# rahulaggarwal965/vslam

Measured on AMD Instinct MI355X. Metric: frame-pairs/sec (extract+match+RANSAC) @1280×720, 2k kp, 4096 hyp; 1/2/4/8 GPU, higher is better.
Workload: dtype u8/f32/f64; 1 GPU; C3: 1280x720, 2000 keypoints, 4096 hypotheses, batch 256 pairs per GPU, SURVEY 8(d) data: rotation + parallax, sub-pixel resampling, 40-45 % outlier matches; pairs_per_gpu=256, batches_in_flight=4

## Files before the change

vslam_amd/build.py:

```python
import os
import subprocess
import sys

HERE = os.path.dirname(os.path.abspath(__file__))
CSRC = os.path.join(HERE, "csrc")
LIB = os.path.join(HERE, "libvslam_amd.so")
SOURCES = ["capi.hip", "match.hip", "ransac_sets.hip", "ransac_solve.hip", "ransac_count.hip", "ransac_prune.hip", "ransac_select.hip", "refit.hip", "refine.hip",
           "kdtree.hip", "gray.hip", "response.hip", "select.hip", "blur.hip",
           "brief.hip", "orb_grid.hip", "pose.hip", "assoc.hip", "map.hip", "world.hip", "resect.hip", "adjust.hip", "search.hip", "render.hip", "multi.hip", "pipeline.hip"]
HEADERS = ["ctx.h", "introselect.h", "image_common.h", "ransac_svd.h", "ransac_residual.h", "ransac_prune_cert.h", "block_reduce.h", "lm_math.h", "refine_math.h", "resect_math.h", "adjust_math.h", "search_math.h", "world_select.h", "world_match.h",
           os.path.join("..", "..", "include", "vslam_amd.h"),
           os.path.join("..", "..", "include", "vslam_resect.h"),
           os.path.join("..", "..", "include", "vslam_adjust.h"),
           os.path.join("..", "..", "include", "vslam_search.h"),
           os.path.join("..", "..", "include", "vslam_brief_pattern_31.h")]
FLAGS = ["--offload-arch=gfx950", "-O3", "-std=c++17", "-ffp-contract=off", "-fPIC", "-Wall"]
EXTRA_FLAGS = {"response.hip": ["-fno-slp-vectorize"]}
OBJDIR = os.path.join(HERE, "_obj")


EXP_LIB = os.path.join(HERE, "libvslam_amd_exp.so")
EXP_OBJDIR = os.path.join(HERE, "_obj_exp")


def _compile(hipcc, src, verbose, objdir=None, extra=()):
# ... 64 lines not shown
```

vslam_amd/capi.py:

```python
import ctypes as C
import os

_HERE = os.path.dirname(os.path.abspath(__file__))
LIB_PATH = os.environ.get("VSLAM_AMD_LIB") or os.path.join(_HERE, "libvslam_amd.so")
EXP_LIB_PATH = os.path.join(_HERE, "libvslam_amd_exp.so")

OK = 0
ERRORS = {-1: "VSLAM_ERR_INVALID", -2: "VSLAM_ERR_HIP", -3: "VSLAM_ERR_NO_DEVICE",
          -4: "VSLAM_ERR_CAPACITY", -5: "VSLAM_ERR_DEGENERATE", -6: "VSLAM_ERR_COMM"}

SYMBOLS = [
    "vslam_ctx_create", "vslam_ctx_make_current", "vslam_ctx_destroy", "vslam_ctx_set_stream", "vslam_ctx_set_option", "vslam_ctx_synchronize", "vslam_ctx_wait",
    "vslam_last_error", "vslam_ctx_workspace_bytes", "vslam_version", "vslam_brief_pattern_31", "vslam_dev_alloc", "vslam_dev_free", "vslam_copy_h2d",
    "vslam_copy_d2h", "vslam_debug_stream_copy", "vslam_debug_valu_calib", "vslam_prof_enable", "vslam_prof_reset", "vslam_prof_count", "vslam_prof_get",
    "vslam_match_knn2_ratio", "vslam_ransac_sets", "vslam_ransac_fundamental", "vslam_ransac_solve",
    "vslam_ransac_evaluate", "vslam_refit_fundamental", "vslam_refine_pairs", "vslam_kdtree_build",
    "vslam_kdtree_radius", "vslam_kdtree_nearest", "vslam_kdtree_cell_table", "vslam_extract_features", "vslam_extract_features_grid", "vslam_triangulate_points", "vslam_frontend_pairs_pose", "vslam_pipeline_batches_redone", "vslam_corner_stats", "vslam_bgr2gray", "vslam_min_eigen",
    "vslam_good_features", "vslam_gaussian7", "vslam_orb_describe", "vslam_extract_Rt", "vslam_triangulate", "vslam_associate_map_points", "vslam_reprojection_filter",
    "vslam_match_features",
    "vslam_map_create", "vslam_map_destroy", "vslam_map_reset", "vslam_map_step", "vslam_map_view", "vslam_map_observations",
    "vslam_track_sequences",
    "vslam_world_create", "vslam_world_destroy", "vslam_world_reset", "vslam_world_step", "vslam_world_lift", "vslam_world_view",
    "vslam_map_attach_world", "vslam_world_render",
    "vslam_view_default", "vslam_view_look_at", "vslam_render_points", "vslam_map_render",
# ... 255 lines not shown
        W = width if width is not None else bgr.shape[2]
        stride = bgr.shape[2] * (bgr.shape[3] if bgr.dim() == 4 else 1)
        xy = torch.zeros((F, max_corners, 2), dtype=torch.float32, device=bgr.device)
        n = torch.zeros((F,), dtype=torch.int32, device=bgr.device)
        self._ready()
        self._check(self.lib.vslam_debug_detect(self.handle, _ptr(bgr), C.c_int(F), C.c_int(W), C.c_int(H), C.c_int(stride),
                                                C.c_int(max_corners), C.c_int(max_corners), _ptr(xy), _ptr(n)))
        return xy, n

    def debug_ransac_prune_x(self, batch, hyp):
        torch = self.torch
        x = torch.zeros((batch, hyp), dtype=torch.int32, device="cuda")
        self._ready()
        self._check(self.lib.vslam_debug_ransac_prune_x(self.handle, _ptr(x), C.c_int(batch), C.c_int(hyp)))
        return x

    def debug_ransac_prune_tile(self, F, xy):
        torch = self.torch
        self._dev(F, torch.float32, "F"); self._dev(xy, torch.float32, "xy")
        assert tuple(F.shape) == (32, 9) and tuple(xy.shape) == (4, 32)
        n = torch.zeros((32, 32), dtype=torch.float32, device=F.device)
        a0 = torch.zeros((32, 32), dtype=torch.float32, device=F.device)
        self._ready()
        self._check(self.lib.vslam_debug_ransac_prune_tile(self.handle, _ptr(F), _ptr(xy), _ptr(n), _ptr(a0)))
        return n, a0

    def debug_valu_calib(self):
        self._check(self.lib.vslam_debug_valu_calib(self.handle))

    def debug_stream_copy(self, src, dst, bytes_per_lane):
# ... 1016 lines not shown
```

vslam_amd/csrc/match.hip:

```cpp
#include "ctx.h"

#include <cstdlib>

namespace {

constexpr int kThreads = 256;
#ifdef VSLAM_EXPERIMENTS
constexpr int kQueriesPerLane = 2;
constexpr int kTile = 256;

__device__ __forceinline__ uint32_t bcnt_acc(uint32_t x, uint32_t acc) {
    uint32_t r;
    asm("v_bcnt_u32_b32 %0, %1, %2" : "=v"(r) : "v"(x), "v"(acc));
    return r;
}
__device__ __forceinline__ uint32_t med3_u32(uint32_t a, uint32_t b, uint32_t c) {
    uint32_t r;
    asm("v_med3_u32 %0, %1, %2, %3" : "=v"(r) : "v"(a), "v"(b), "v"(c));
    return r;
}
__device__ __forceinline__ uint32_t ham256(const uint4 &qa, const uint4 &qb, const uint4 &ta,
                                           const uint4 &tb) {
    uint32_t d = bcnt_acc(qa.x ^ ta.x, 0u);
    d = bcnt_acc(qa.y ^ ta.y, d);
// ... 265 lines not shown
                int4 o;
                o.x = nt >= 1 ? i0 : -1;
                o.y = nt >= 1 ? d0 : 0x7FFFFFFF;
                o.z = nt >= 2 ? i1 : -1;
                o.w = nt >= 2 ? d1 : 0x7FFFFFFF;
                knn_b[q] = o;
            }
        }
}

#endif

typedef int v8i __attribute__((ext_vector_type(8)));
typedef float v16f __attribute__((ext_vector_type(16)));
constexpr int kFStride = 144;
constexpr float kFScale = 16384.f;
constexpr float kFPad = 33554432.f;
constexpr float kFNone = -67108864.f;
constexpr int kFBias = 0x05000000;

__device__ __forceinline__ uint32_t spread8_pm1(uint32_t b) {
    uint32_t x = (b | (b << 12)) & 0x000F000Fu;
    x = (x | (x << 6)) & 0x03030303u;
    x = (x | (x << 3)) & 0x11111111u;
    return (x << 3) | 0x22222222u;
}
__device__ __forceinline__ v4i spread32_pm1(uint32_t w) {
    v4i r;
    r.x = (int)spread8_pm1(w & 0xFFu);
    r.y = (int)spread8_pm1((w >> 8) & 0xFFu);
    r.z = (int)spread8_pm1((w >> 16) & 0xFFu);
    r.w = (int)spread8_pm1(w >> 24);
    return r;
}
__device__ __forceinline__ float med3_f32(float a, float b, float c) { return __builtin_amdgcn_fmed3f(a, b, c); }

__global__ __launch_bounds__(256) void match_spread_kernel(const uint8_t *__restrict__ desc2, const int32_t *__restrict__ n2,
                                                           int kp_stride, int kp_pad, uint8_t *__restrict__ tx) {
    const int b = blockIdx.y, i = blockIdx.x * 256 + threadIdx.x;
    const int row = i >> 3;
    if (row >= n2[b]) return;
    const uint32_t w = reinterpret_cast<const uint32_t *>(desc2 + (size_t)b * kp_stride * VSLAM_DESC_BYTES)[i];
    *reinterpret_cast<v4i *>(tx + ((size_t)b * kp_pad + row) * 128 + (size_t)(i & 7) * 16) = spread32_pm1(w);
}

template <int RT, bool PRE, int CT>
__global__ __launch_bounds__(64 * kMQ / (32 * RT)) void match_knn2_fp4_kernel(
    const uint8_t *__restrict__ desc1, const int32_t *__restrict__ n1, const uint8_t *__restrict__ desc2,
    const int32_t *__restrict__ n2, int kp_stride, int32_t *__restrict__ sel, int32_t *__restrict__ knn,
    const uint8_t *__restrict__ tx, int kp_pad, int batch, int per_pair) {
    int b, qt;
    vs_xcd_item_block(blockIdx.x, per_pair, b, qt);
    if (b >= batch) return;
    const int tid = threadIdx.x, lane = tid & 63;
    const int wave = __builtin_amdgcn_readfirstlane(tid >> 6);
    const int nq = n1[b], nt = n2[b];
    const int qbase = qt * kMQ;
    if (qbase >= nq) return;

    static_assert(CT == 1 || PRE, "two tiles per trip only with pre-spread train rows");
    __shared__ __align__(16) uint8_t s_b[2][CT * kMT * kFStride];
    const uint32_t *q32 = reinterpret_cast<const uint32_t *>(desc1 + (size_t)b * kp_stride * VSLAM_DESC_BYTES);
    const uint32_t *t32 = reinterpret_cast<const uint32_t *>(desc2 + (size_t)b * kp_stride * VSLAM_DESC_BYTES);
    int32_t *sel_b = sel + (size_t)b * kp_stride;
    int4 *knn_b = knn ? reinterpret_cast<int4 *>(knn) + (size_t)b * kp_stride : nullptr;

    const int r = lane & 31, half = lane >> 5;
    v8i a[RT][4];
#pragma unroll
    for (int rt = 0; rt < RT; rt++) {
        const int q = min(qbase + wave * (32 * RT) + rt * 32 + r, nq - 1);
        const uint2 *qrow = reinterpret_cast<const uint2 *>(q32 + (size_t)q * 8);
#pragma unroll
        for (int s = 0; s < 4; s++) {
            const uint2 w2 = qrow[s];
            const v4i x = spread32_pm1(half ? w2.y : w2.x);
// ... 2 lines not shown
    }
    float k1[RT][16], k2[RT][16];
#pragma unroll
    for (int rt = 0; rt < RT; rt++)
#pragma unroll
        for (int g = 0; g < 16; g++) {
            k1[rt][g] = kFNone;
            k2[rt][g] = kFNone;
        }

    constexpr bool kSplit = RT == 1;
    const int st = kSplit ? (tid & 255) : tid, shalf = kSplit ? (tid >> 8) : 0;
    const int srow = st >> 3, sd = st & 7;
    struct Stage {
        uint4 v[CT];
    };
    const uint8_t *txb = PRE ? tx + (size_t)b * kp_pad * 128 + (size_t)srow * 128 + sd * 16 + (kSplit ? 8 * shalf : 0) : nullptr;
    auto fetch = [&](int trip) -> Stage {
        Stage st_;
#pragma unroll
        for (int c = 0; c < CT; c++) {
            uint4 v = make_uint4(0u, 0u, 0u, 0u);
            if (PRE) {
                const uint8_t *src = txb + (size_t)(trip * CT + c) * (kMT * 128);
                if (kSplit) {
                    const uint2 h = *reinterpret_cast<const uint2 *>(src);
                    v.x = h.x;
                    v.y = h.y;
                } else {
                    v = *reinterpret_cast<const uint4 *>(src);
                }
            } else {
                const int t = trip * kMT + srow;
                v.x = t < nt ? t32[(size_t)t * 8 + sd] : 0u;
            }
            st_.v[c] = v;
        }
        return st_;
    };
    auto expand = [&](const Stage &st_, int buf) {
#pragma unroll
        for (int c = 0; c < CT; c++) {
            const uint4 v = st_.v[c];
            uint8_t *dst = &s_b[buf][(c * kMT + srow) * kFStride + sd * 16];
            if (PRE) {
                if (kSplit) *reinterpret_cast<uint2 *>(dst + 8 * shalf) = make_uint2(v.x, v.y);
                else *reinterpret_cast<uint4 *>(dst) = v;
            } else if (kSplit) {
                const uint32_t hw = (v.x >> (16 * shalf)) & 0xFFFFu;
                *reinterpret_cast<uint2 *>(dst + 8 * shalf) = make_uint2(spread8_pm1(hw & 0xFFu), spread8_pm1(hw >> 8));
            } else {
                *reinterpret_cast<v4i *>(dst) = spread32_pm1(v.x);
            }
        }
    };

    const int ntrips = (nt + CT * kMT - 1) / (CT * kMT);
    if (ntrips > 0) expand(fetch(0), 0);
    Stage w_next;
    if (ntrips > 1) w_next = fetch(1);
    __syncthreads();
    for (int trip = 0; trip < ntrips; trip++) {
        const int buf = trip & 1;
        if (trip + 1 < ntrips) expand(w_next, buf ^ 1);
        if (trip + 2 < ntrips) w_next = fetch(trip + 2);
        v16f acc[CT][RT];
#pragma unroll
        for (int c = 0; c < CT; c++) {
#pragma unroll
            for (int rt = 0; rt < RT; rt++) acc[c][rt] = v16f{0, 0, 0, 0, 0, 0, 0, 0, 0, 0, 0, 0, 0, 0, 0, 0};
            const uint8_t *src = &s_b[buf][(c * kMT + r) * kFStride + 16 * half];
#pragma unroll
            for (int s = 0; s < 4; s++) {
                const v4i bq = *reinterpret_cast<const v4i *>(src + 32 * s);
                const v8i bv = v8i{bq.x, bq.y, bq.z, bq.w, 0, 0, 0, 0};
#pragma unroll
                for (int rt = 0; rt < RT; rt++)
                    acc[c][rt] = __builtin_amdgcn_mfma_scale_f32_32x32x64_f8f6f4(a[rt][s], bv, acc[c][rt], 4, 4, 0, 0x7F7F7F7F, 0, 0x7F7F7F7F);
            }
        }
#pragma unroll
        for (int c = 0; c < CT; c++) {
            const int t = (trip * CT + c) * kMT + r;
            const float nidx = t < nt ? -(float)t : -kFPad;
#pragma unroll
            for (int g = 0; g < 16; g++) {
#pragma unroll
                for (int rt = 0; rt < RT; rt++) {
                    const float key = __builtin_fmaf(acc[c][rt][g], kFScale, nidx);
                    k2[rt][g] = med3_f32(k1[rt][g], k2[rt][g], key);
                    k1[rt][g] = fmaxf(k1[rt][g], key);
                }
            }
        }
        __syncthreads();
    }

#pragma unroll
    for (int rt = 0; rt < RT; rt++)
#pragma unroll
        for (int g = 0; g < 16; g++) {
            uint32_t x1 = (uint32_t)(kFBias - (int)k1[rt][g]), x2 = (uint32_t)(kFBias - (int)k2[rt][g]);
            merge2<0xB1>(x1, x2);
            merge2<0x4E>(x1, x2);
// ... 70 lines not shown
                    const int32_t *n2, int batch, int kp_stride, int32_t *pairs, int32_t *m,
                    int32_t *knn) {
    VS_REQUIRE(ctx, d1 && n1 && d2 && n2 && pairs && m, VSLAM_ERR_INVALID);
    VS_REQUIRE(ctx, batch > 0 && kp_stride > 0, VSLAM_ERR_INVALID);
    VS_REQUIRE(ctx, kp_stride <= VSLAM_MAX_KP, VSLAM_ERR_CAPACITY);
    int32_t *sel = nullptr;
    int rc = vs_arena_get(ctx, "match.sel", sizeof(int32_t) * (size_t)batch * kp_stride, (void **)&sel);
    if (rc) return rc;
#ifndef VSLAM_EXPERIMENTS
    {
        VsProfScope ps(ctx, "match_knn2_kernel");
        const int per_pair = vs_div_up(kp_stride, kMQ);
        const int xgrid = vs_xcd_grid(batch, per_pair);
        const int kp_pad = vs_div_up(kp_stride, 2 * kMT) * 2 * kMT;
        uint8_t *tx = nullptr;
        if ((rc = vs_arena_get(ctx, "match.spread", (size_t)batch * kp_pad * 128, (void **)&tx))) return rc;
        match_spread_kernel<<<dim3(vs_div_up(kp_stride * 8, 256), batch), 256, 0, ctx->stream>>>(d2, n2, kp_stride, kp_pad, tx);
        match_knn2_fp4_kernel<1, true, 2><<<xgrid, 512, 0, ctx->stream>>>(d1, n1, d2, n2, kp_stride, sel, knn, tx, kp_pad, batch, per_pair);
    }
#else
    static const bool popcount_path = VS_EXPERIMENT_ENV("VSLAM_MATCH_POPCOUNT") != nullptr;
    {
        VsProfScope ps(ctx, "match_knn2_kernel");
        if (popcount_path) {
            dim3 grid(vs_div_up(kp_stride, kThreads * kQueriesPerLane), batch);
            match_knn2_kernel<<<grid, kThreads, 0, ctx->stream>>>(d1, n1, d2, n2, kp_stride, sel, knn);
        } else {
            static const char *const shape = VS_EXPERIMENT_ENV("VSLAM_MATCH_SHAPE");
#ifdef VSLAM_EXPERIMENTS
            const int pick = ctx->match_shape ? ctx->match_shape : (shape ? (shape[0] == '4' ? 2 : 1) : 0);
#else
            constexpr int pick = 0;
            (void)shape;
// ... 2 lines not shown
            dim3 grid(vs_div_up(kp_stride, kMQ), batch);
            static const char *const form = VS_EXPERIMENT_ENV("VSLAM_MATCH_FORM");
#ifdef VSLAM_EXPERIMENTS
            const bool fp4 = ctx->match_form ? ctx->match_form == 1 : !(form && form[0] == 'i');
#else
            constexpr bool fp4 = true;
            (void)form;
#endif
            if (fp4) {
                const bool wide4 = pick == 2;
                const int per_pair = vs_div_up(kp_stride, kMQ);
                const int xgrid = vs_xcd_grid(batch, per_pair);
                static const char *const nopre = VS_EXPERIMENT_ENV("VSLAM_MATCH_NO_PRESPREAD");
                static const char *const ct_env = VS_EXPERIMENT_ENV("VSLAM_MATCH_TILES_PER_TRIP");
                const int ct = ct_env ? atoi(ct_env) : 2;
                if (!nopre) {
                    const int kp_pad = vs_div_up(kp_stride, 2 * kMT) * 2 * kMT;
                    uint8_t *tx = nullptr;
                    if ((rc = vs_arena_get(ctx, "match.spread", (size_t)batch * kp_pad * 128, (void **)&tx))) return rc;
                    match_spread_kernel<<<dim3(vs_div_up(kp_stride * 8, 256), batch), 256, 0, ctx->stream>>>(d2, n2, kp_stride, kp_pad, tx);
                    if (wide4 && ct == 2) match_knn2_fp4_kernel<2, true, 2><<<xgrid, 256, 0, ctx->stream>>>(d1, n1, d2, n2, kp_stride, sel, knn, tx, kp_pad, batch, per_pair);
                    else if (wide4) match_knn2_fp4_kernel<2, true, 1><<<xgrid, 256, 0, ctx->stream>>>(d1, n1, d2, n2, kp_stride, sel, knn, tx, kp_pad, batch, per_pair);
                    else if (ct == 2) match_knn2_fp4_kernel<1, true, 2><<<xgrid, 512, 0, ctx->stream>>>(d1, n1, d2, n2, kp_stride, sel, knn, tx, kp_pad, batch, per_pair);
                    else match_knn2_fp4_kernel<1, true, 1><<<xgrid, 512, 0, ctx->stream>>>(d1, n1, d2, n2, kp_stride, sel, knn, tx, kp_pad, batch, per_pair);
                } else if (wide4) {
                    match_knn2_fp4_kernel<2, false, 1><<<xgrid, 256, 0, ctx->stream>>>(d1, n1, d2, n2, kp_stride, sel, knn, nullptr, 0, batch, per_pair);
                } else {
                    match_knn2_fp4_kernel<1, false, 1><<<xgrid, 512, 0, ctx->stream>>>(d1, n1, d2, n2, kp_stride, sel, knn, nullptr, 0, batch, per_pair);
                }
            } else if (wide) match_knn2_mfma_kernel<2><<<grid, 256, 0, ctx->stream>>>(d1, n1, d2, n2, kp_stride, sel, knn);
            else match_knn2_mfma_kernel<1><<<grid, 512, 0, ctx->stream>>>(d1, n1, d2, n2, kp_stride, sel, knn);
        }
    }
#endif
    {
        VsProfScope ps(ctx, "match_compact_kernel");
        match_compact_kernel<<<batch, kThreads, 0, ctx->stream>>>(sel, n1, kp_stride, pairs, m);
    }
    VS_HIP(ctx, hipGetLastError());
    return VSLAM_OK;
}
```

vslam_amd/csrc/ransac_count.hip:

```cpp
#include "ransac_residual.h"

namespace {
using namespace vs_ransac;

constexpr int kCntHyps = 128;
constexpr int kCntWaves = 8;
constexpr int kCntQueue = 320;
constexpr int kCntLdsMatches = 4096;
constexpr int kScreenMatches = 128;
constexpr int kScreenHyps = 128;
constexpr int kRankThreads = 512;
constexpr int kPilotHyps = kRankThreads / 64;
constexpr int kCandMax = 8;
constexpr float kCntTinyDD = 0x1p-120f;
constexpr int kFcmpOGT = 2, kFcmpOLT = 4, kFcmpULT = 12;
constexpr int kCntRec = 12;
typedef __attribute__((address_space(3))) volatile uint32_t cnt_queue_t;
static_assert(VSLAM_MAX_KP <= 65536, "queue words keep the match index in 16 bits");

__host__ __device__ constexpr int cnt_pad(int n) { return (n + 255) & ~255; }
constexpr int kHeadUncertified = -1;
__device__ __forceinline__ float cnt_sum_rel(int adds) { return fmaxf(0x1p-18f, (float)(13 + adds) * 0x1p-24f); }

struct CntBand {
    float lo, hi;
    double beta;
    bool ok;
};
__device__ __forceinline__ CntBand cnt_band(const float *f, float C1, float C2, float threshold) {
    CntBand B;
    bool ok = threshold >= 0x1p-20f && threshold <= 0x1p20f && C1 <= 0x1p20f && C2 <= 0x1p20f;
#pragma unroll
    for (int k = 0; k < 9; k++) ok = ok && fabsf(f[k]) <= 1024.f;
    const double S = ((double)fabsf(f[0]) + (double)fabsf(f[3]) + (double)fabsf(f[1]) + (double)fabsf(f[4])) * (double)C2 +
                     (double)fabsf(f[6]) + (double)fabsf(f[7]);
    const double beta = 4.04 * 0x1p-24 * S + 1e-30;
// ... 317 lines not shown
            r[2 * kp_pad + pos] = c.x;
            r[3 * kp_pad + pos] = c.y;
        }
    }
    const int mpad = cnt_pad(m);
    if (m + tid < mpad) {
        const int2 pr = PR[m - 1];
        const float2 a = P1[pr.x], c = P2[pr.y];
        r[m + tid] = a.x;
        r[kp_pad + m + tid] = a.y;
        r[2 * kp_pad + m + tid] = c.x;
        r[3 * kp_pad + m + tid] = c.y;
    }
}

__global__ __launch_bounds__(256) void ransac_screen_kernel(
    const float *__restrict__ rk, int kp_pad, const int32_t *__restrict__ m_arr, int min_m, int kp_stride, int hyp,
    float threshold, const float *__restrict__ hypF, const float *__restrict__ cmax, const int32_t *__restrict__ cbound,
    int32_t *__restrict__ pot0, int2 *__restrict__ head) {
    const int b = blockIdx.y, tid = threadIdx.x, lane = tid & 63;
    const int wave = __builtin_amdgcn_readfirstlane(tid >> 6);
    const int hbase = blockIdx.x * kScreenHyps;
    const int m = min(m_arr[b], kp_stride);
    if (m < min_m) return;
    __shared__ __align__(16) float s_rec[kScreenHyps * kCntRec];
    if (tid < kScreenHyps) {
        const float *src = hypF + ((size_t)b * hyp + min(hbase + tid, hyp - 1)) * 9;
        float f[9];
#pragma unroll
        for (int k = 0; k < 9; k++) f[k] = src[k];
        const CntBand B = cnt_band(f, cmax[2 * b], cmax[2 * b + 1], threshold);
        cnt_store_record(s_rec + tid * kCntRec, f, B);
    }
    const int n0 = min(m, kScreenMatches);
    const int bound_pilots = cbound[b];
    const float *r = rk + (size_t)b * 4 * kp_pad;
    const float2 x1 = *reinterpret_cast<const float2 *>(r + 2 * lane);
    const float2 y1 = *reinterpret_cast<const float2 *>(r + kp_pad + 2 * lane);
    const float2 x2 = *reinterpret_cast<const float2 *>(r + 2 * kp_pad + 2 * lane);
    const float2 y2 = *reinterpret_cast<const float2 *>(r + 3 * kp_pad + 2 * lane);
    v2f X1, Y1, X2, Y2;
    X1.x = x1.x; X1.y = x1.y; Y1.x = y1.x; Y1.y = y1.y;
    X2.x = x2.x; X2.y = x2.y; Y2.x = y2.x; Y2.y = y2.y;
    const unsigned long long va = __ballot(2 * lane < n0), vb = __ballot(2 * lane + 1 < n0);
    __syncthreads();
    int mine = 0;
    float mine_sum = 0.f;
    const bool odd1 = (lane & 1) != 0, odd2 = (lane & 2) != 0;
    const bool in_a = 2 * lane < n0, in_b = 2 * lane + 1 < n0;
    constexpr int kU = 4;
// ... 411 lines not shown
    const bool from_zero = VS_EXPERIMENT_ENV("VSLAM_RANSAC_COUNT_FROM_ZERO") != nullptr;
#ifdef VSLAM_EXPERIMENTS
    const int exit_payload = VS_EXPERIMENT_ENV("VSLAM_RANSAC_COUNT_EXIT_PAYLOAD") != nullptr ? 1 : 0;
#endif
    int2 *head = nullptr;
    if ((rc = vs_arena_get(ctx, "ransac.head", sizeof(int2) * (size_t)batch * hyp, (void **)&head))) return rc;
    const unsigned long long *use_floor = no_sum_rule ? nullptr : sfloor;
    if ((rc = vs_arena_get(ctx, "ransac.pot0", sizeof(int32_t) * (size_t)batch * hyp, (void **)&pot0))) return rc;
    if ((rc = vs_arena_get(ctx, "ransac.rk", sizeof(float) * 4 * (size_t)kp_pad * batch, (void **)&rk))) return rc;
    if ((rc = vs_arena_get(ctx, "ransac.cmax", sizeof(float) * 2 * (size_t)batch, (void **)&cmax))) return rc;
    {
        VsProfScope ps(ctx, "ransac_rank_kernel");
        ransac_rank_kernel<<<batch, kRankThreads, 0, ctx->stream>>>(xy1, xy2, pairs, m, min_m, kp_stride, kp_pad, hyp, threshold, hypF,
                                                                    cbound, rk, cmax, sfloor);
    }
    {
        VsProfScope ps(ctx, "ransac_screen_kernel");
        dim3 grid(vs_div_up(hyp, kScreenHyps), batch);
        ransac_screen_kernel<<<grid, 256, 0, ctx->stream>>>(rk, kp_pad, m, min_m, kp_stride, hyp, threshold, hypF, cmax, cbound, pot0, head);
    }
    {
        VsProfScope ps(ctx, "ransac_cand_kernel");
        ransac_cand_kernel<<<batch, 64 * kCandMax, 0, ctx->stream>>>(rk, kp_pad, m, min_m, kp_stride, hyp, threshold, hypF, pot0,
                                                                     no_sum_rule ? 0 : 1, cbound, sfloor);
    }
    if ((rc = vs_launch_ransac_prune(ctx, rk, kp_pad, m, min_m, kp_stride, hyp, threshold, hypF, cmax, cbound, pot0, batch, kScreenMatches)))
        return rc;
    if (int arc = vs_aux_job_point(ctx, 4)) return arc;
    {
        VsProfScope ps(ctx, "ransac_count_kernel");
        const bool lds = kp_pad <= kCntLdsMatches;
        const size_t dyn = (lds ? sizeof(float) * 4 * (size_t)kp_pad : 0) + sizeof(uint32_t) * kCntQueue * kCntWaves;
        const size_t dyn_max = sizeof(float) * 4 * kCntLdsMatches + sizeof(uint32_t) * kCntQueue * kCntWaves;
        dim3 grid(vs_div_up(hyp, kCntHyps), batch);
#ifdef VSLAM_EXPERIMENTS
// ... 30 lines not shown
```

vslam_amd/csrc/ransac_prune.hip:

```cpp
#include "ransac_prune_cert.h"
#include "ransac_residual.h"

namespace {

typedef float v16f __attribute__((ext_vector_type(16)));
constexpr int kPruneWaves = 4;
constexpr int kPruneHyps = 32;
constexpr int kPruneTile = 32;
constexpr int kPruneStep = 2;
constexpr int kPruneOGT = 2;

__host__ __device__ constexpr int prune_row(int r, int half) { return (r & 3) + 8 * (r >> 2) + 4 * half; }

struct PruneA {
    float n[5], d[2];
};
__device__ __forceinline__ PruneA prune_operands(const float *f, bool half) {
    PruneA A;
#pragma unroll
    for (int s = 0; s < 4; s++) A.n[s] = half ? f[2 * s + 1] : f[2 * s];
    A.n[4] = half ? 0.f : f[8];
    A.d[0] = half ? f[1] : f[0];
    A.d[1] = half ? 0.f : f[2];
    return A;
}

__device__ __forceinline__ void prune_tile(const PruneA &A, bool half, float x1, float y1, float x2, float y2, v16f &n, v16f &a0) {
    const float p = x2 * (half ? y1 : x1);
    const float q = y2 * (half ? x1 : y1);
    const float b1 = half ? q : x2, b2 = half ? y2 : q, b3 = half ? y1 : x1, b4 = half ? 0.f : 1.f;
    v16f z;
#pragma unroll
    for (int r = 0; r < 16; r++) z[r] = 0.f;
    n = __builtin_amdgcn_mfma_f32_32x32x2f32(A.n[0], p, z, 0, 0, 0);
    n = __builtin_amdgcn_mfma_f32_32x32x2f32(A.n[1], b1, n, 0, 0, 0);
    n = __builtin_amdgcn_mfma_f32_32x32x2f32(A.n[2], b2, n, 0, 0, 0);
    n = __builtin_amdgcn_mfma_f32_32x32x2f32(A.n[3], b3, n, 0, 0, 0);
    n = __builtin_amdgcn_mfma_f32_32x32x2f32(A.n[4], b4, n, 0, 0, 0);
    a0 = __builtin_amdgcn_mfma_f32_32x32x2f32(A.d[0], b3, z, 0, 0, 0);
    a0 = __builtin_amdgcn_mfma_f32_32x32x2f32(A.d[1], b4, a0, 0, 0, 0);
}

#ifdef VSLAM_EXPERIMENTS
#define VS_PRUNE_X_PARAM , int32_t *__restrict__ x_out
#else
#define VS_PRUNE_X_PARAM
#endif

__global__ __launch_bounds__(64 * kPruneWaves) void ransac_prune_mfma_kernel(
    const float *__restrict__ rk, int kp_pad, const int32_t *__restrict__ m_arr, int min_m, int kp_stride, int hyp, float threshold,
    float splus, const float *__restrict__ hypF, const float *__restrict__ cmax, const int32_t *__restrict__ cbound, int32_t *__restrict__ pot0,
    int n_head, int gate VS_PRUNE_X_PARAM) {
    const int b = blockIdx.y, lane = threadIdx.x & 63, col = lane & 31;
    const bool half = lane >= 32;
    const int wave = __builtin_amdgcn_readfirstlane(threadIdx.x >> 6);
    const int m = min(m_arr[b], kp_stride);
// ... 113 lines not shown
#endif
    return VSLAM_OK;
}

#ifdef VSLAM_EXPERIMENTS
extern "C" {
int vslam_debug_ransac_prune_x(vslam_ctx *ctx, int32_t *d_out, int batch, int hyp) {
    if (!ctx) return VSLAM_ERR_INVALID;
    VS_REQUIRE(ctx, d_out && batch > 0 && hyp > 0 && vs_ptr_bits(d_out) % 4 == 0, VSLAM_ERR_INVALID);
    const size_t bytes = sizeof(int32_t) * (size_t)batch * hyp;
    const auto it = ctx->arena.find("ransac.prune_x");
    VS_REQUIRE(ctx, it != ctx->arena.end() && it->second.bytes >= bytes, VSLAM_ERR_INVALID);
    VS_HIP(ctx, hipMemcpyAsync(d_out, it->second.ptr, bytes, hipMemcpyDeviceToDevice, ctx->stream));
    return VSLAM_OK;
}
int vslam_debug_ransac_prune_tile(vslam_ctx *ctx, const float *d_F, const float *d_xy, float *d_n, float *d_a0) {
    if (!ctx) return VSLAM_ERR_INVALID;
    VS_REQUIRE(ctx, d_F && d_xy && d_n && d_a0 && vs_ptr_bits(d_F, d_xy, d_n, d_a0) % 4 == 0, VSLAM_ERR_INVALID);
    ransac_prune_tile_kernel<<<1, 64, 0, ctx->stream>>>(d_F, d_xy, d_n, d_a0);
    return VSLAM_OK;
}
}
#endif
```

vslam_amd/csrc/ransac_residual.h:

```cpp
#pragma once

#include "ctx.h"

namespace vs_ransac {

struct ResidualF {
    float f[9];
    double ft[6];
};
__device__ __forceinline__ void residual_prepare(ResidualF &R) {
    R.ft[0] = (double)R.f[0];
    R.ft[1] = (double)R.f[3];
    R.ft[2] = (double)R.f[6];
    R.ft[3] = (double)R.f[1];
    R.ft[4] = (double)R.f[4];
    R.ft[5] = (double)R.f[7];
}
__device__ __forceinline__ float residual_e(const ResidualF &R, const float4 c, const double dx2, const double dy2) {
    const float x1 = c.x, y1 = c.y, x2 = c.z, y2 = c.w;
    const float a0 = R.f[0] * x1 + R.f[1] * y1 + R.f[2];
    const float a1 = R.f[3] * x1 + R.f[4] * y1 + R.f[5];
    const float a2 = R.f[6] * x1 + R.f[7] * y1 + R.f[8];
    const float t0 = (float)(__builtin_fma(R.ft[1], dy2, R.ft[0] * dx2) + R.ft[2]);
    const float t1 = (float)(__builtin_fma(R.ft[4], dy2, R.ft[3] * dx2) + R.ft[5]);
// ... 18 lines not shown
    v2f q;
    q.x = nn.x / dd.x;
    q.y = nn.y / dd.y;
    return ((q + a1 * a1) + t0 * t0) + t1 * t1;
}

}

int vs_launch_ransac_count(vslam_ctx *ctx, const float *xy1, const float *xy2, const int32_t *pairs, const int32_t *m,
                           const float *hypF, int batch, int kp_stride, int hyp, float threshold, int32_t *hyp_count,
                           float *hyp_sum, float *approx);

int vs_launch_ransac_prune(vslam_ctx *ctx, const float *rk, int kp_pad, const int32_t *m, int min_m, int kp_stride, int hyp,
                           float threshold, const float *hypF, const float *cmax, const int32_t *cbound, int32_t *pot0, int batch,
                           int n_head);
```

Before: 102,500 frame-pairs/s.

## Add certificate-based MFMA head screening route and alternate fp4 match key forms

```diff
diff --git a/vslam_amd/build.py b/vslam_amd/build.py
--- a/vslam_amd/build.py
+++ b/vslam_amd/build.py
@@ -8,7 +8,7 @@
 SOURCES = ["capi.hip", "match.hip", "ransac_sets.hip", "ransac_solve.hip", "ransac_count.hip", "ransac_prune.hip", "ransac_select.hip", "refit.hip", "refine.hip",
            "kdtree.hip", "gray.hip", "response.hip", "select.hip", "blur.hip",
            "brief.hip", "orb_grid.hip", "pose.hip", "assoc.hip", "map.hip", "world.hip", "resect.hip", "adjust.hip", "search.hip", "render.hip", "multi.hip", "pipeline.hip"]
-HEADERS = ["ctx.h", "introselect.h", "image_common.h", "ransac_svd.h", "ransac_residual.h", "ransac_prune_cert.h", "block_reduce.h", "lm_math.h", "refine_math.h", "resect_math.h", "adjust_math.h", "search_math.h", "world_select.h", "world_match.h",
+HEADERS = ["ctx.h", "introselect.h", "image_common.h", "ransac_svd.h", "ransac_residual.h", "ransac_prune_cert.h", "ransac_prune_tile.h", "block_reduce.h", "lm_math.h", "refine_math.h", "resect_math.h", "adjust_math.h", "search_math.h", "world_select.h", "world_match.h",
            os.path.join("..", "..", "include", "vslam_amd.h"),
            os.path.join("..", "..", "include", "vslam_resect.h"),
            os.path.join("..", "..", "include", "vslam_adjust.h"),
diff --git a/vslam_amd/capi.py b/vslam_amd/capi.py
--- a/vslam_amd/capi.py
+++ b/vslam_amd/capi.py
@@ -293,6 +293,14 @@
         self._ready()
         self._check(self.lib.vslam_debug_ransac_prune_x(self.handle, _ptr(x), C.c_int(batch), C.c_int(hyp)))
         return x
+
+    def debug_ransac_head(self, batch, hyp):
+        torch = self.torch
+        pot0 = torch.zeros((batch, hyp), dtype=torch.int32, device="cuda")
+        route = torch.zeros((batch,), dtype=torch.int32, device="cuda")
+        self._ready()
+        self._check(self.lib.vslam_debug_ransac_head(self.handle, _ptr(pot0), _ptr(route), C.c_int(batch), C.c_int(hyp)))
+        return pot0, route
 
     def debug_ransac_prune_tile(self, F, xy):
         torch = self.torch
diff --git a/vslam_amd/csrc/match.hip b/vslam_amd/csrc/match.hip
--- a/vslam_amd/csrc/match.hip
+++ b/vslam_amd/csrc/match.hip
@@ -303,6 +303,11 @@
 typedef int v8i __attribute__((ext_vector_type(8)));
 typedef float v16f __attribute__((ext_vector_type(16)));
 constexpr int kFStride = 144;
+constexpr int kFKeyForm = 0;
+constexpr int kFRowBytes2 = 160;
+constexpr int kFStride2 = 176;
+constexpr int kFScale7 = 0x86868686;
+constexpr int kFScale0 = 0x7F7F7F7F;
 constexpr float kFScale = 16384.f;
 constexpr float kFPad = 33554432.f;
 constexpr float kFNone = -67108864.f;
@@ -323,17 +328,34 @@
     return r;
 }
 __device__ __forceinline__ float med3_f32(float a, float b, float c) { return __builtin_amdgcn_fmed3f(a, b, c); }
-
+__device__ __forceinline__ v4i index_chunk(int v) {
+    const int q = v / 6, rem = v - 6 * q;
+    const uint32_t code = (0x00EEDCA0u >> (4 * rem)) & 0xFu, extra = rem == 5 ? 0xAu : 0u;
+    uint32_t w[4];
+#pragma unroll
+    for (int k = 0; k < 4; k++) {
+        const int n = min(max(q - 8 * k, 0), 8);
+        w[k] = n == 8 ? 0xFFFFFFFFu : (1u << (4 * n)) - 1u;
+        if ((q >> 3) == k) w[k] |= code << (4 * (q & 7));
+        if (((q + 1) >> 3) == k) w[k] |= extra << (4 * ((q + 1) & 7));
+    }
+    return v4i{(int)w[0], (int)w[1], (int)w[2], (int)w[3]};
+}
+
+template <bool IDX>
 __global__ __launch_bounds__(256) void match_spread_kernel(const uint8_t *__restrict__ desc2, const int32_t *__restrict__ n2,
                                                            int kp_stride, int kp_pad, uint8_t *__restrict__ tx) {
+    constexpr int kRow = IDX ? kFRowBytes2 : 128;
     const int b = blockIdx.y, i = blockIdx.x * 256 + threadIdx.x;
     const int row = i >> 3;
     if (row >= n2[b]) return;
     const uint32_t w = reinterpret_cast<const uint32_t *>(desc2 + (size_t)b * kp_stride * VSLAM_DESC_BYTES)[i];
-    *reinterpret_cast<v4i *>(tx + ((size_t)b * kp_pad + row) * 128 + (size_t)(i & 7) * 16) = spread32_pm1(w);
-}
-
-template <int RT, bool PRE, int CT>
+    uint8_t *dst = tx + ((size_t)b * kp_pad + row) * kRow;
+    *reinterpret_cast<v4i *>(dst + (size_t)(i & 7) * 16) = spread32_pm1(w);
+    if (IDX && (i & 7) < 2) *reinterpret_cast<v4i *>(dst + 128 + 16 * (i & 7)) = index_chunk((i & 7) ? row >> 7 : row & 127);
+}
+
+template <int RT, bool PRE, int CT, int KF>
 __global__ __launch_bounds__(64 * kMQ / (32 * RT)) void match_knn2_fp4_kernel(
     const uint8_t *__restrict__ desc1, const int32_t *__restrict__ n1, const uint8_t *__restrict__ desc2,
     const int32_t *__restrict__ n2, int kp_stride, int32_t *__restrict__ sel, int32_t *__restrict__ knn,
@@ -348,7 +370,11 @@
     if (qbase >= nq) return;
 
     static_assert(CT == 1 || PRE, "two tiles per trip only with pre-spread train rows");
-    __shared__ __align__(16) uint8_t s_b[2][CT * kMT * kFStride];
+    static_assert(KF >= 0 && KF <= 3 && (KF != 2 || PRE), "the index chunks come from match_spread_kernel");
+    static_assert(VSLAM_MAX_KP <= 16384, "index chunks: index >> 7 <= 127");
+    constexpr int kStride = KF == 2 ? kFStride2 : kFStride, kRow = KF == 2 ? kFRowBytes2 : 128;
+    constexpr int kScale = KF == 0 ? kFScale0 : kFScale7;
+    __shared__ __align__(16) uint8_t s_b[2][CT * kMT * kStride];
     const uint32_t *q32 = reinterpret_cast<const uint32_t *>(desc1 + (size_t)b * kp_stride * VSLAM_DESC_BYTES);
     const uint32_t *t32 = reinterpret_cast<const uint32_t *>(desc2 + (size_t)b * kp_stride * VSLAM_DESC_BYTES);
     int32_t *sel_b = sel + (size_t)b * kp_stride;
@@ -381,15 +407,18 @@
     const int srow = st >> 3, sd = st & 7;
     struct Stage {
         uint4 v[CT];
+        uint4 x;
     };
-    const uint8_t *txb = PRE ? tx + (size_t)b * kp_pad * 128 + (size_t)srow * 128 + sd * 16 + (kSplit ? 8 * shalf : 0) : nullptr;
+    const uint8_t *txb = PRE ? tx + (size_t)b * kp_pad * kRow + (size_t)srow * kRow + sd * 16 + (kSplit ? 8 * shalf : 0) : nullptr;
+    const bool xmine = KF == 2 && wave < CT;
+    const int xoff = (wave * kMT + (lane >> 1)), xb = 128 + 16 * (lane & 1);
     auto fetch = [&](int trip) -> Stage {
         Stage st_;
 #pragma unroll
         for (int c = 0; c < CT; c++) {
             uint4 v = make_uint4(0u, 0u, 0u, 0u);
             if (PRE) {
-                const uint8_t *src = txb + (size_t)(trip * CT + c) * (kMT * 128);
+                const uint8_t *src = txb + (size_t)(trip * CT + c) * (kMT * kRow);
                 if (kSplit) {
                     const uint2 h = *reinterpret_cast<const uint2 *>(src);
                     v.x = h.x;
@@ -403,13 +432,15 @@
             }
             st_.v[c] = v;
         }
+        st_.x = make_uint4(0u, 0u, 0u, 0u);
+        if (xmine) st_.x = *reinterpret_cast<const uint4 *>(tx + ((size_t)b * kp_pad + (size_t)trip * CT * kMT + xoff) * kRow + xb);
         return st_;
     };
     auto expand = [&](const Stage &st_, int buf) {
 #pragma unroll
         for (int c = 0; c < CT; c++) {
             const uint4 v = st_.v[c];
-            uint8_t *dst = &s_b[buf][(c * kMT + srow) * kFStride + sd * 16];
+            uint8_t *dst = &s_b[buf][(c * kMT + srow) * kStride + sd * 16];
             if (PRE) {
                 if (kSplit) *reinterpret_cast<uint2 *>(dst + 8 * shalf) = make_uint2(v.x, v.y);
                 else *reinterpret_cast<uint4 *>(dst) = v;
@@ -420,6 +451,7 @@
                 *reinterpret_cast<v4i *>(dst) = spread32_pm1(v.x);
             }
         }
+        if (xmine) *reinterpret_cast<uint4 *>(&s_b[buf][xoff * kStride + xb]) = st_.x;
     };
 
     const int ntrips = (nt + CT * kMT - 1) / (CT * kMT);
@@ -432,29 +464,58 @@
         if (trip + 1 < ntrips) expand(w_next, buf ^ 1);
         if (trip + 2 < ntrips) w_next = fetch(trip + 2);
         v16f acc[CT][RT];
+        float nidx[CT];
 #pragma unroll
         for (int c = 0; c < CT; c++) {
-#pragma unroll
-            for (int rt = 0; rt < RT; rt++) acc[c][rt] = v16f{0, 0, 0, 0, 0, 0, 0, 0, 0, 0, 0, 0, 0, 0, 0, 0};
-            const uint8_t *src = &s_b[buf][(c * kMT + r) * kFStride + 16 * half];
+            const int t = (trip * CT + c) * kMT + r;
+            nidx[c] = t < nt ? -(float)t : -kFPad;
+        }
+#pragma unroll
+        for (int c = 0; c < CT; c++) {
+#pragma unroll
+            for (int rt = 0; rt < RT; rt++) {
+                if (KF == 3) {
+#pragma unroll
+                    for (int g = 0; g < 16; g++) acc[c][rt][g] = nidx[c];
+                } else {
+                    acc[c][rt] = v16f{0, 0, 0, 0, 0, 0, 0, 0, 0, 0, 0, 0, 0, 0, 0, 0};
+                }
+            }
+            const uint8_t *src = &s_b[buf][(c * kMT + r) * kStride + 16 * half];
 #pragma unroll
             for (int s = 0; s < 4; s++) {
                 const v4i bq = *reinterpret_cast<const v4i *>(src + 32 * s);
                 const v8i bv = v8i{bq.x, bq.y, bq.z, bq.w, 0, 0, 0, 0};
 #pragma unroll
                 for (int rt = 0; rt < RT; rt++)
-                    acc[c][rt] = __builtin_amdgcn_mfma_scale_f32_32x32x64_f8f6f4(a[rt][s], bv, acc[c][rt], 4, 4, 0, 0x7F7F7F7F, 0, 0x7F7F7F7F);
-            }
+                    acc[c][rt] = __builtin_amdgcn_mfma_scale_f32_32x32x64_f8f6f4(a[rt][s], bv, acc[c][rt], 4, 4, 0, kScale, 0, kScale);
+            }
+            if (KF == 2) {
+                const v4i bq = *reinterpret_cast<const v4i *>(src + 128);
+                const v8i bv = v8i{bq.x, bq.y, bq.z, bq.w, 0, 0, 0, 0};
+                const v8i ones = v8i{0x22222222, 0x22222222, 0x22222222, 0x22222222, 0, 0, 0, 0};
+                const int sidx = half ? kFScale7 : kFScale0;
+#pragma unroll
+                for (int rt = 0; rt < RT; rt++)
+                    acc[c][rt] = __builtin_amdgcn_mfma_scale_f32_32x32x64_f8f6f4(ones, bv, acc[c][rt], 4, 4, 0, kFScale0, 0, sidx);
+            }
+        }
+        if (KF == 2 && trip == ntrips - 1) {
+#pragma unroll
+            for (int c = 0; c < CT; c++)
+#pragma unroll
+                for (int rt = 0; rt < RT; rt++)
+#pragma unroll
+                    for (int g = 0; g < 16; g++) acc[c][rt][g] = nidx[c] == -kFPad ? kFNone : acc[c][rt][g];
         }
 #pragma unroll
         for (int c = 0; c < CT; c++) {
-            const int t = (trip * CT + c) * kMT + r;
-            const float nidx = t < nt ? -(float)t : -kFPad;
 #pragma unroll
             for (int g = 0; g < 16; g++) {
 #pragma unroll
                 for (int rt = 0; rt < RT; rt++) {
-                    const float key = __builtin_fmaf(acc[c][rt][g], kFScale, nidx);
+                    const float key = KF == 0 ? __builtin_fmaf(acc[c][rt][g], kFScale, nidx[c])
+                                              : (KF == 1 ? acc[c][rt][g] + nidx[c] : acc[c][rt][g]);
                     k2[rt][g] = med3_f32(k1[rt][g], k2[rt][g], key);
                     k1[rt][g] = fmaxf(k1[rt][g], key);
                 }
@@ -555,9 +616,10 @@
         const int xgrid = vs_xcd_grid(batch, per_pair);
         const int kp_pad = vs_div_up(kp_stride, 2 * kMT) * 2 * kMT;
         uint8_t *tx = nullptr;
-        if ((rc = vs_arena_get(ctx, "match.spread", (size_t)batch * kp_pad * 128, (void **)&tx))) return rc;
-        match_spread_kernel<<<dim3(vs_div_up(kp_stride * 8, 256), batch), 256, 0, ctx->stream>>>(d2, n2, kp_stride, kp_pad, tx);
-        match_knn2_fp4_kernel<1, true, 2><<<xgrid, 512, 0, ctx->stream>>>(d1, n1, d2, n2, kp_stride, sel, knn, tx, kp_pad, batch, per_pair);
+        constexpr bool kIdx = kFKeyForm == 2;
+        if ((rc = vs_arena_get(ctx, "match.spread", (size_t)batch * kp_pad * (kIdx ? kFRowBytes2 : 128), (void **)&tx))) return rc;
+        match_spread_kernel<kIdx><<<dim3(vs_div_up(kp_stride * 8, 256), batch), 256, 0, ctx->stream>>>(d2, n2, kp_stride, kp_pad, tx);
+        match_knn2_fp4_kernel<1, true, 2, kFKeyForm><<<xgrid, 512, 0, ctx->stream>>>(d1, n1, d2, n2, kp_stride, sel, knn, tx, kp_pad, batch, per_pair);
     }
 #else
     static const bool popcount_path = VS_EXPERIMENT_ENV("VSLAM_MATCH_POPCOUNT") != nullptr;
@@ -590,20 +652,36 @@
                 static const char *const nopre = VS_EXPERIMENT_ENV("VSLAM_MATCH_NO_PRESPREAD");
                 static const char *const ct_env = VS_EXPERIMENT_ENV("VSLAM_MATCH_TILES_PER_TRIP");
                 const int ct = ct_env ? atoi(ct_env) : 2;
+                const char *const kf_env = VS_EXPERIMENT_ENV("VSLAM_MATCH_KEY_FORM");
+                const int kf = kf_env ? atoi(kf_env) : kFKeyForm;
+                VS_REQUIRE(ctx, kf >= 0 && kf <= 3, VSLAM_ERR_INVALID);
+#define VS_FP4_LAUNCH(RT_, PRE_, CT_, KF_, THREADS_, TX_, PAD_) \
+    match_knn2_fp4_kernel<RT_, PRE_, CT_, KF_><<<xgrid, THREADS_, 0, ctx->stream>>>(d1, n1, d2, n2, kp_stride, sel, knn, TX_, PAD_, batch, per_pair)
+#define VS_FP4_FORMS(RT_, PRE_, CT_, THREADS_, TX_, PAD_)                                  \
+    do {                                                                                   \
+        if (kf == 0) VS_FP4_LAUNCH(RT_, PRE_, CT_, 0, THREADS_, TX_, PAD_);                \
+        else if (kf == 3) VS_FP4_LAUNCH(RT_, PRE_, CT_, 3, THREADS_, TX_, PAD_);           \
+        else if (kf == 2 && PRE_) VS_FP4_LAUNCH(RT_, PRE_, CT_, (PRE_ ? 2 : 1), THREADS_, TX_, PAD_); \
+        else VS_FP4_LAUNCH(RT_, PRE_, CT_, 1, THREADS_, TX_, PAD_);                        \
+    } while (0)
                 if (!nopre) {
                     const int kp_pad = vs_div_up(kp_stride, 2 * kMT) * 2 * kMT;
                     uint8_t *tx = nullptr;
-                    if ((rc = vs_arena_get(ctx, "match.spread", (size_t)batch * kp_pad * 128, (void **)&tx))) return rc;
-                    match_spread_kernel<<<dim3(vs_div_up(kp_stride * 8, 256), batch), 256, 0, ctx->stream>>>(d2, n2, kp_stride, kp_pad, tx);
-                    if (wide4 && ct == 2) match_knn2_fp4_kernel<2, true, 2><<<xgrid, 256, 0, ctx->stream>>>(d1, n1, d2, n2, kp_stride, sel, knn, tx, kp_pad, batch, per_pair);
-                    else if (wide4) match_knn2_fp4_kernel<2, true, 1><<<xgrid, 256, 0, ctx->stream>>>(d1, n1, d2, n2, kp_stride, sel, knn, tx, kp_pad, batch, per_pair);
-                    else if (ct == 2) match_knn2_fp4_kernel<1, true, 2><<<xgrid, 512, 0, ctx->stream>>>(d1, n1, d2, n2, kp_stride, sel, knn, tx, kp_pad, batch, per_pair);
-                    else match_knn2_fp4_kernel<1, true, 1><<<xgrid, 512, 0, ctx->stream>>>(d1, n1, d2, n2, kp_stride, sel, knn, tx, kp_pad, batch, per_pair);
+                    if ((rc = vs_arena_get(ctx, "match.spread", (size_t)batch * kp_pad * kFRowBytes2, (void **)&tx))) return rc;
+                    const dim3 sgrid(vs_div_up(kp_stride * 8, 256), batch);
+                    if (kf == 2) match_spread_kernel<true><<<sgrid, 256, 0, ctx->stream>>>(d2, n2, kp_stride, kp_pad, tx);
+                    else match_spread_kernel<false><<<sgrid, 256, 0, ctx->stream>>>(d2, n2, kp_stride, kp_pad, tx);
+                    if (wide4 && ct == 2) VS_FP4_FORMS(2, true, 2, 256, tx, kp_pad);
+                    else if (wide4) VS_FP4_FORMS(2, true, 1, 256, tx, kp_pad);
+                    else if (ct == 2) VS_FP4_FORMS(1, true, 2, 512, tx, kp_pad);
+                    else VS_FP4_FORMS(1, true, 1, 512, tx, kp_pad);
                 } else if (wide4) {
-                    match_knn2_fp4_kernel<2, false, 1><<<xgrid, 256, 0, ctx->stream>>>(d1, n1, d2, n2, kp_stride, sel, knn, nullptr, 0, batch, per_pair);
+                    VS_FP4_FORMS(2, false, 1, 256, nullptr, 0);
                 } else {
-                    match_knn2_fp4_kernel<1, false, 1><<<xgrid, 512, 0, ctx->stream>>>(d1, n1, d2, n2, kp_stride, sel, knn, nullptr, 0, batch, per_pair);
+                    VS_FP4_FORMS(1, false, 1, 512, nullptr, 0);
                 }
+#undef VS_FP4_FORMS
+#undef VS_FP4_LAUNCH
             } else if (wide) match_knn2_mfma_kernel<2><<<grid, 256, 0, ctx->stream>>>(d1, n1, d2, n2, kp_stride, sel, knn);
             else match_knn2_mfma_kernel<1><<<grid, 512, 0, ctx->stream>>>(d1, n1, d2, n2, kp_stride, sel, knn);
         }
diff --git a/vslam_amd/csrc/ransac_count.hip b/vslam_amd/csrc/ransac_count.hip
--- a/vslam_amd/csrc/ransac_count.hip
+++ b/vslam_amd/csrc/ransac_count.hip
@@ -1,3 +1,4 @@
+#include "ransac_prune_tile.h"
 #include "ransac_residual.h"
 
 namespace {
@@ -19,7 +20,7 @@
 static_assert(VSLAM_MAX_KP <= 65536, "queue words keep the match index in 16 bits");
 
 __host__ __device__ constexpr int cnt_pad(int n) { return (n + 255) & ~255; }
-constexpr int kHeadUncertified = -1;
+constexpr int kHeadUncertified = kVsHeadUncertified;
 __device__ __forceinline__ float cnt_sum_rel(int adds) { return fmaxf(0x1p-18f, (float)(13 + adds) * 0x1p-24f); }
 
 struct CntBand {
@@ -367,15 +368,32 @@
     }
 }
 
-__global__ __launch_bounds__(256) void ransac_screen_kernel(
+#ifdef VSLAM_EXPERIMENTS
+#define VS_SCREEN_ROUTE_PARAM , int32_t *__restrict__ route_out
+#else
+#define VS_SCREEN_ROUTE_PARAM
+#endif
+__global__ __launch_bounds__(256) __attribute__((amdgpu_waves_per_eu(7, 7))) void ransac_screen_kernel(
     const float *__restrict__ rk, int kp_pad, const int32_t *__restrict__ m_arr, int min_m, int kp_stride, int hyp,
     float threshold, const float *__restrict__ hypF, const float *__restrict__ cmax, const int32_t *__restrict__ cbound,
-    int32_t *__restrict__ pot0, int2 *__restrict__ head) {
+    int32_t *__restrict__ pot0, int2 *__restrict__ head, float splus, int route VS_SCREEN_ROUTE_PARAM) {
     const int b = blockIdx.y, tid = threadIdx.x, lane = tid & 63;
     const int wave = __builtin_amdgcn_readfirstlane(tid >> 6);
     const int hbase = blockIdx.x * kScreenHyps;
     const int m = min(m_arr[b], kp_stride);
+    const int bound_pilots = cbound[b];
+#ifdef VSLAM_EXPERIMENTS
+    if (route_out && blockIdx.x == 0 && tid == 0)
+        route_out[b] = m < min_m ? -1 : (vs_head_on_certificate(m, bound_pilots, min(m, kScreenMatches), route) ? 1 : 0);
+#endif
     if (m < min_m) return;
+    if (vs_head_on_certificate(m, bound_pilots, min(m, kScreenMatches), route)) {
+        static_assert(kScreenHyps == vs_prune::kPruneWaves * vs_prune::kPruneHyps && kScreenMatches <= vs_prune::kHeadTiles * vs_prune::kPruneTile,
+                      "a wave of the screen is a wave of the prune tile");
+        if (hbase + wave * 32 < hyp)
+            vs_prune::head_on_certificate(rk, kp_pad, b, m, min(m, kScreenMatches), hbase + wave * 32, hyp, threshold, splus, hypF, cmax, pot0, head);
+        return;
+    }
     __shared__ __align__(16) float s_rec[kScreenHyps * kCntRec];
     if (tid < kScreenHyps) {
         const float *src = hypF + ((size_t)b * hyp + min(hbase + tid, hyp - 1)) * 9;
@@ -386,7 +404,6 @@
         cnt_store_record(s_rec + tid * kCntRec, f, B);
     }
     const int n0 = min(m, kScreenMatches);
-    const int bound_pilots = cbound[b];
     const float *r = rk + (size_t)b * 4 * kp_pad;
     const float2 x1 = *reinterpret_cast<const float2 *>(r + 2 * lane);
     const float2 y1 = *reinterpret_cast<const float2 *>(r + kp_pad + 2 * lane);
@@ -828,11 +845,27 @@
         ransac_rank_kernel<<<batch, kRankThreads, 0, ctx->stream>>>(xy1, xy2, pairs, m, min_m, kp_stride, kp_pad, hyp, threshold, hypF,
                                                                     cbound, rk, cmax, sfloor);
     }
+    int route = -1;
+    if (const char *e = VS_EXPERIMENT_ENV("VSLAM_RANSAC_HEAD_ROUTE")) route = atoi(e) ? 1 : 0;
+#ifdef VSLAM_EXPERIMENTS
+    int32_t *route_out = nullptr, *pot0_out = nullptr;
+    if ((rc = vs_arena_get(ctx, "ransac.head_route", sizeof(int32_t) * (size_t)batch, (void **)&route_out))) return rc;
+    if ((rc = vs_arena_get(ctx, "ransac.head_pot0", sizeof(int32_t) * (size_t)batch * hyp, (void **)&pot0_out))) return rc;
+#endif
     {
         VsProfScope ps(ctx, "ransac_screen_kernel");
         dim3 grid(vs_div_up(hyp, kScreenHyps), batch);
-        ransac_screen_kernel<<<grid, 256, 0, ctx->stream>>>(rk, kp_pad, m, min_m, kp_stride, hyp, threshold, hypF, cmax, cbound, pot0, head);
-    }
+#ifdef VSLAM_EXPERIMENTS
+        ransac_screen_kernel<<<grid, 256, 0, ctx->stream>>>(rk, kp_pad, m, min_m, kp_stride, hyp, threshold, hypF, cmax, cbound, pot0, head,
+                                                            pc_splus(threshold), route, route_out);
+#else
+        ransac_screen_kernel<<<grid, 256, 0, ctx->stream>>>(rk, kp_pad, m, min_m, kp_stride, hyp, threshold, hypF, cmax, cbound, pot0, head,
+                                                            pc_splus(threshold), route);
+#endif
+    }
+#ifdef VSLAM_EXPERIMENTS
+    VS_HIP(ctx, hipMemcpyAsync(pot0_out, pot0, sizeof(int32_t) * (size_t)batch * hyp, hipMemcpyDeviceToDevice, ctx->stream));
+#endif
     {
         VsProfScope ps(ctx, "ransac_cand_kernel");
         ransac_cand_kernel<<<batch, 64 * kCandMax, 0, ctx->stream>>>(rk, kp_pad, m, min_m, kp_stride, hyp, threshold, hypF, pot0,
diff --git a/vslam_amd/csrc/ransac_prune.hip b/vslam_amd/csrc/ransac_prune.hip
--- a/vslam_amd/csrc/ransac_prune.hip
+++ b/vslam_amd/csrc/ransac_prune.hip
@@ -1,45 +1,9 @@
-#include "ransac_prune_cert.h"
-#include "ransac_residual.h"
+#include "ransac_prune_tile.h"
 
 namespace {
+using namespace vs_prune;
 
-typedef float v16f __attribute__((ext_vector_type(16)));
-constexpr int kPruneWaves = 4;
-constexpr int kPruneHyps = 32;
-constexpr int kPruneTile = 32;
 constexpr int kPruneStep = 2;
-constexpr int kPruneOGT = 2;
-
-__host__ __device__ constexpr int prune_row(int r, int half) { return (r & 3) + 8 * (r >> 2) + 4 * half; }
-
-struct PruneA {
-    float n[5], d[2];
-};
-__device__ __forceinline__ PruneA prune_operands(const float *f, bool half) {
-    PruneA A;
-#pragma unroll
-    for (int s = 0; s < 4; s++) A.n[s] = half ? f[2 * s + 1] : f[2 * s];
-    A.n[4] = half ? 0.f : f[8];
-    A.d[0] = half ? f[1] : f[0];
-    A.d[1] = half ? 0.f : f[2];
-    return A;
-}
-
-__device__ __forceinline__ void prune_tile(const PruneA &A, bool half, float x1, float y1, float x2, float y2, v16f &n, v16f &a0) {
-    const float p = x2 * (half ? y1 : x1);
-    const float q = y2 * (half ? x1 : y1);
-    const float b1 = half ? q : x2, b2 = half ? y2 : q, b3 = half ? y1 : x1, b4 = half ? 0.f : 1.f;
-    v16f z;
-#pragma unroll
-    for (int r = 0; r < 16; r++) z[r] = 0.f;
-    n = __builtin_amdgcn_mfma_f32_32x32x2f32(A.n[0], p, z, 0, 0, 0);
-    n = __builtin_amdgcn_mfma_f32_32x32x2f32(A.n[1], b1, n, 0, 0, 0);
-    n = __builtin_amdgcn_mfma_f32_32x32x2f32(A.n[2], b2, n, 0, 0, 0);
-    n = __builtin_amdgcn_mfma_f32_32x32x2f32(A.n[3], b3, n, 0, 0, 0);
-    n = __builtin_amdgcn_mfma_f32_32x32x2f32(A.n[4], b4, n, 0, 0, 0);
-    a0 = __builtin_amdgcn_mfma_f32_32x32x2f32(A.d[0], b3, z, 0, 0, 0);
-    a0 = __builtin_amdgcn_mfma_f32_32x32x2f32(A.d[1], b4, a0, 0, 0, 0);
-}
 
 #ifdef VSLAM_EXPERIMENTS
 #define VS_PRUNE_X_PARAM , int32_t *__restrict__ x_out
@@ -183,6 +147,17 @@
     VS_HIP(ctx, hipMemcpyAsync(d_out, it->second.ptr, bytes, hipMemcpyDeviceToDevice, ctx->stream));
     return VSLAM_OK;
 }
+int vslam_debug_ransac_head(vslam_ctx *ctx, int32_t *d_pot0, int32_t *d_route, int batch, int hyp) {
+    if (!ctx) return VSLAM_ERR_INVALID;
+    VS_REQUIRE(ctx, d_pot0 && d_route && batch > 0 && hyp > 0 && vs_ptr_bits(d_pot0, d_route) % 4 == 0, VSLAM_ERR_INVALID);
+    const size_t bytes = sizeof(int32_t) * (size_t)batch * hyp;
+    const auto ip = ctx->arena.find("ransac.head_pot0"), ir = ctx->arena.find("ransac.head_route");
+    VS_REQUIRE(ctx, ip != ctx->arena.end() && ip->second.bytes >= bytes, VSLAM_ERR_INVALID);
+    VS_REQUIRE(ctx, ir != ctx->arena.end() && ir->second.bytes >= sizeof(int32_t) * (size_t)batch, VSLAM_ERR_INVALID);
+    VS_HIP(ctx, hipMemcpyAsync(d_pot0, ip->second.ptr, bytes, hipMemcpyDeviceToDevice, ctx->stream));
+    VS_HIP(ctx, hipMemcpyAsync(d_route, ir->second.ptr, sizeof(int32_t) * (size_t)batch, hipMemcpyDeviceToDevice, ctx->stream));
+    return VSLAM_OK;
+}
 int vslam_debug_ransac_prune_tile(vslam_ctx *ctx, const float *d_F, const float *d_xy, float *d_n, float *d_a0) {
     if (!ctx) return VSLAM_ERR_INVALID;
     VS_REQUIRE(ctx, d_F && d_xy && d_n && d_a0 && vs_ptr_bits(d_F, d_xy, d_n, d_a0) % 4 == 0, VSLAM_ERR_INVALID);
diff --git a/vslam_amd/csrc/ransac_prune_tile.h b/vslam_amd/csrc/ransac_prune_tile.h
--- /dev/null
+++ b/vslam_amd/csrc/ransac_prune_tile.h
@@ -0,0 +1,98 @@
+#pragma once
+
+#include "ransac_prune_cert.h"
+#include "ransac_residual.h"
+
+namespace vs_prune {
+
+typedef float v16f __attribute__((ext_vector_type(16)));
+constexpr int kPruneWaves = 4;
+constexpr int kPruneHyps = 32;
+constexpr int kPruneTile = 32;
+constexpr int kPruneOGT = 2;
+
+__host__ __device__ constexpr int prune_row(int r, int half) { return (r & 3) + 8 * (r >> 2) + 4 * half; }
+
+struct PruneA {
+    float n[5], d[2];
+};
+__device__ __forceinline__ PruneA prune_operands(const float *f, bool half) {
+    PruneA A;
+#pragma unroll
+    for (int s = 0; s < 4; s++) A.n[s] = half ? f[2 * s + 1] : f[2 * s];
+    A.n[4] = half ? 0.f : f[8];
+    A.d[0] = half ? f[1] : f[0];
+    A.d[1] = half ? 0.f : f[2];
+    return A;
+}
+
+__device__ __forceinline__ void prune_tile(const PruneA &A, bool half, float x1, float y1, float x2, float y2, v16f &n, v16f &a0) {
+    const float p = x2 * (half ? y1 : x1);
+    const float q = y2 * (half ? x1 : y1);
+    const float b1 = half ? q : x2, b2 = half ? y2 : q, b3 = half ? y1 : x1, b4 = half ? 0.f : 1.f;
+    v16f z;
+#pragma unroll
+    for (int r = 0; r < 16; r++) z[r] = 0.f;
+    n = __builtin_amdgcn_mfma_f32_32x32x2f32(A.n[0], p, z, 0, 0, 0);
+    n = __builtin_amdgcn_mfma_f32_32x32x2f32(A.n[1], b1, n, 0, 0, 0);
+    n = __builtin_amdgcn_mfma_f32_32x32x2f32(A.n[2], b2, n, 0, 0, 0);
+    n = __builtin_amdgcn_mfma_f32_32x32x2f32(A.n[3], b3, n, 0, 0, 0);
+    n = __builtin_amdgcn_mfma_f32_32x32x2f32(A.n[4], b4, n, 0, 0, 0);
+    a0 = __builtin_amdgcn_mfma_f32_32x32x2f32(A.d[0], b3, z, 0, 0, 0);
+    a0 = __builtin_amdgcn_mfma_f32_32x32x2f32(A.d[1], b4, a0, 0, 0, 0);
+}
+
+constexpr int kHeadTiles = 4;
+__device__ __forceinline__ void head_on_certificate(const float *__restrict__ rk, int kp_pad, int b, int m, int n0, int hbase, int hyp,
+                                                    float threshold, float splus, const float *__restrict__ hypF,
+                                                    const float *__restrict__ cmax, int32_t *__restrict__ pot0, int2 *__restrict__ head) {
+    const int lane = threadIdx.x & 63, col = lane & 31;
+    const bool half = lane >= 32;
+    const int h = hbase + col;
+    const size_t hi = (size_t)b * hyp + min(h, hyp - 1);
+    float f[9];
+#pragma unroll
+    for (int k = 0; k < 9; k++) f[k] = hypF[hi * 9 + k];
+    const float c = pc_margin(f, cmax[2 * b], cmax[2 * b + 1], threshold, splus);
+    const PruneA A = prune_operands(f, half);
+    float cr[16];
+#pragma unroll
+    for (int r = 0; r < 16; r++) cr[r] = __shfl(c, half ? prune_row(r, 1) : prune_row(r, 0), 64);
+
+    const float *r1 = rk + (size_t)b * 4 * kp_pad, *r2 = r1 + kp_pad, *r3 = r2 + kp_pad, *r4 = r3 + kp_pad;
+    float x1[kHeadTiles], y1[kHeadTiles], x2[kHeadTiles], y2[kHeadTiles];
+#pragma unroll
+    for (int t = 0; t < kHeadTiles; t++) {
+        const int j = min(t * kPruneTile + col, m - 1);
+        x1[t] = r1[j];
+        y1[t] = r2[j];
+        x2[t] = r3[j];
+        y2[t] = r4[j];
+    }
+    int X[kPruneHyps];
+#pragma unroll
+    for (int i = 0; i < kPruneHyps; i++) X[i] = 0;
+#pragma unroll
+    for (int t = 0; t < kHeadTiles; t++) {
+        if (t * kPruneTile >= n0) break;
+        v16f n, a0;
+        prune_tile(A, half, x1[t], y1[t], x2[t], y2[t], n, a0);
+        const unsigned long long valid = __ballot(t * kPruneTile + col < n0);
+#pragma unroll
+        for (int r = 0; r < 16; r++) {
+            const unsigned long long miss =
+                __builtin_amdgcn_fcmpf(fabsf(n[r]), fmaf(splus, fabsf(a0[r]), cr[r]), kPruneOGT) & valid;
+            X[prune_row(r, 0)] += __popc((uint32_t)miss);
+            X[prune_row(r, 1)] += __popc((uint32_t)(miss >> 32));
+        }
+    }
+    int xv = 0;
+#pragma unroll
+    for (int i = 0; i < kPruneHyps; i++) xv = col == i ? X[i] : xv;
+    if (!half && h < hyp) {
+        pot0[hi] = n0 - xv;
+        head[hi] = make_int2(kVsHeadUncertified, 0);
+    }
+}
+
+}
diff --git a/vslam_amd/csrc/ransac_residual.h b/vslam_amd/csrc/ransac_residual.h
--- a/vslam_amd/csrc/ransac_residual.h
+++ b/vslam_amd/csrc/ransac_residual.h
@@ -56,3 +56,9 @@
 int vs_launch_ransac_prune(vslam_ctx *ctx, const float *rk, int kp_pad, const int32_t *m, int min_m, int kp_stride, int hyp,
                            float threshold, const float *hypF, const float *cmax, const int32_t *cbound, int32_t *pot0, int batch,
                            int n_head);
+
+constexpr int kVsHeadUncertified = -1;
+
+__host__ __device__ constexpr bool vs_head_on_certificate(int m, int bound, int n0, int route) {
+    return m > 0 && (route < 0 ? m - bound + 1 > n0 : route != 0);
+}
```

Result: faster. 104,100 frame-pairs/s, median of 6 (+1.6%).
